# charleschen003/doudizhu-rl

Measured on AMD Instinct MI355X. Metric: env steps/sec (batched tables), higher is better.
Workload: dtype u8; 1 GPU; 65536 tables per GPU, random policy (engine RNG), legal-move list only (no NN), auto-reset: the workload of BASELINE.json configs[1] at the largest single-GPU table count (65,536 per GPU: configs[2] / configs[3]; configs[4] = 8 x 65,536), the same per-GPU workload at every N; tables_per_gpu=65536, total_tables=65536, episodes=2767981, list_layout=slab (fixed-stride segment per table)

## Files before the change

doudizhu-rl_amd/_lib.py:

```python
import ctypes as C
import os

from .build import LIB as _DEFAULT_LIB, LIB_JK as _JK_LIB

_libs = {}

SYMBOLS = {
    "ddz_abi_version": (C.c_int, []),
    "ddz_num_actions": (C.c_int, []),
    "ddz_strerror": (C.c_char_p, [C.c_int]),
    "ddz_last_hip_error": (C.c_int, []),
    "ddz_state_bytes": (C.c_int64, [C.c_int64]),
    "ddz_scratch_bytes": (C.c_int64, [C.c_int64]),
    "ddz_face_planes": (C.c_int, [C.c_int]),
    "ddz_create": (C.c_int, [C.POINTER(C.c_void_p), C.c_int64, C.c_uint64, C.c_uint64, C.c_int,
                             C.c_void_p, C.c_int64, C.c_void_p, C.c_int64]),
    "ddz_destroy": (C.c_int, [C.c_void_p]),
    "ddz_invalidate": (C.c_int, [C.c_void_p]),
    "ddz_reset": (C.c_int, [C.c_void_p, C.c_void_p, C.c_void_p]),
    "ddz_legal": (C.c_int, [C.c_void_p, C.c_void_p, C.c_void_p, C.c_void_p, C.c_int64, C.c_void_p]),
    "ddz_step": (C.c_int, [C.c_void_p, C.c_int, C.c_void_p, C.c_void_p, C.c_void_p, C.c_int,
                           C.c_void_p, C.c_void_p, C.c_void_p, C.c_void_p, C.c_void_p]),
    "ddz_mask_words": (C.c_int, []),
    "ddz_legal_mask": (C.c_int, [C.c_void_p, C.c_void_p, C.c_void_p]),
# ... 54 lines not shown
    "ddz_q_features_needed": (C.c_int, [C.c_int, C.c_void_p, C.c_int64, C.c_int, C.c_void_p, C.c_void_p, C.c_void_p, C.c_void_p,
                                        C.c_void_p, C.c_void_p, C.c_int64, C.c_void_p]),
    "ddz_q_fc1_dense": (C.c_int, [C.c_int, C.c_void_p, C.c_int64, C.c_int64, C.c_void_p, C.c_void_p, C.c_void_p]),
    "ddz_q_fc1_rows": (C.c_int, [C.c_int, C.c_void_p, C.c_void_p, C.c_void_p, C.c_void_p, C.c_void_p, C.c_void_p, C.c_int64,
                                 C.c_void_p]),
    "ddz_q_slab_needed": (C.c_int, [C.c_void_p, C.c_void_p, C.c_void_p, C.c_int64, C.c_void_p, C.c_int64, C.c_void_p,
                                    C.c_void_p, C.c_void_p, C.c_void_p, C.c_int64, C.c_void_p, C.c_void_p]),
    "ddz_q_shared_ws_bytes": (C.c_int64, []),
    "ddz_q_shared_need_ws_bytes": (C.c_int64, [C.c_int64]),
    "ddz_q_shared_need": (C.c_int, [C.c_void_p, C.c_void_p, C.c_void_p, C.c_void_p, C.c_int64, C.c_void_p, C.c_int64, C.c_int64,
                                    C.c_void_p, C.c_void_p, C.c_void_p, C.c_void_p, C.c_void_p]),
    "ddz_q_features_drows": (C.c_int, [C.c_int, C.c_void_p, C.c_int64, C.c_int, C.c_void_p, C.c_void_p, C.c_void_p, C.c_void_p,
                                       C.c_int64, C.c_void_p, C.c_void_p, C.c_void_p, C.c_int64, C.c_void_p]),
    "ddz_q_shared_rows": (C.c_int, [C.c_void_p, C.c_void_p, C.c_int64, C.c_int64, C.c_void_p, C.c_void_p, C.c_void_p, C.c_void_p]),
    "ddz_q_shared_hash_ws_bytes": (C.c_int64, [C.c_int64]),
    "ddz_q_shared_rows_hashed": (C.c_int, [C.c_void_p, C.c_int, C.c_void_p, C.c_int64, C.c_int64, C.c_void_p, C.c_void_p, C.c_void_p,
                                           C.c_void_p]),
    "ddz_q_features_rows": (C.c_int, [C.c_int, C.c_void_p, C.c_int64, C.c_int, C.c_void_p, C.c_void_p, C.c_void_p, C.c_void_p,
                                      C.c_void_p, C.c_int64, C.c_int64, C.c_void_p, C.c_void_p, C.c_void_p]),
    "ddz_q_gather_h0": (C.c_int, [C.c_int, C.c_void_p, C.c_int64, C.c_void_p, C.c_int64, C.c_void_p, C.c_void_p, C.c_void_p]),
    "ddz_q_fc1_rows_k": (C.c_int, [C.c_int, C.c_void_p, C.c_int64, C.c_void_p, C.c_void_p, C.c_void_p, C.c_int64, C.c_int, C.c_void_p]),
    "ddz_q_roles_ws_bytes": (C.c_int64, [C.c_int64, C.c_int, C.c_int]),
    "ddz_q_roles_rows": (C.c_int, [C.c_void_p, C.c_int, C.c_void_p, C.c_int, C.c_void_p, C.c_int64, C.c_int64, C.c_void_p, C.c_void_p,
                                   C.c_void_p, C.c_void_p, C.c_void_p]),
    "ddz_q_roles_features_rows": (C.c_int, [C.c_int, C.c_void_p, C.c_int64, C.c_int, C.c_int, C.c_void_p, C.c_void_p, C.c_void_p,
                                            C.c_void_p, C.c_void_p, C.c_int64, C.c_int64, C.c_void_p]),
    "ddz_q_roles_fc1_rows_k": (C.c_int, [C.c_int, C.c_int, C.c_void_p, C.c_int64, C.c_void_p, C.c_void_p, C.c_void_p, C.c_int64,
                                         C.c_void_p]),
    "ddz_q_roles_gather_h0": (C.c_int, [C.c_int, C.c_int, C.c_void_p, C.c_int64, C.c_void_p, C.c_void_p, C.c_int64, C.c_void_p,
                                        C.c_void_p, C.c_void_p]),
    "ddz_q_roles_need_ws_bytes": (C.c_int64, [C.c_int64, C.c_int]),
    "ddz_q_roles_need": (C.c_int, [C.c_void_p, C.c_int, C.c_void_p, C.c_void_p, C.c_void_p, C.c_int64, C.c_void_p, C.c_int64,
                                   C.c_int64, C.c_void_p, C.c_void_p, C.c_void_p, C.c_void_p, C.c_void_p]),
    "ddz_q_roles_features_drows": (C.c_int, [C.c_int, C.c_void_p, C.c_int64, C.c_int, C.c_int, C.c_void_p, C.c_void_p, C.c_void_p,
                                             C.c_void_p, C.c_int64, C.c_void_p, C.c_void_p, C.c_void_p, C.c_int64, C.c_void_p]),
    "ddz_q_roles_fc1_rows": (C.c_int, [C.c_int, C.c_int, C.c_void_p, C.c_void_p, C.c_void_p, C.c_void_p, C.c_void_p, C.c_void_p,
                                       C.c_int64, C.c_void_p]),
    "ddz_q_roles_slab": (C.c_int, [C.c_void_p, C.c_int, C.c_void_p, C.c_void_p, C.c_void_p, C.c_int64, C.c_void_p, C.c_int64,
                                   C.c_void_p, C.c_void_p, C.c_void_p, C.c_void_p, C.c_int64, C.c_void_p, C.c_void_p]),
    "ddz_action_table": (C.c_int, [C.c_int, C.c_void_p, C.c_void_p]),
    "ddz_pack_trajectory": (C.c_int, [C.c_int, C.c_void_p, C.c_int64, C.c_void_p, C.c_void_p]),
    "ddz_auto_choose_state": (C.c_int, [C.c_void_p, C.c_int, C.c_void_p, C.c_void_p, C.c_void_p]),
    "ddz_auto_choose": (C.c_int, [C.c_int, C.c_void_p, C.c_void_p, C.c_void_p, C.c_int64, C.c_void_p, C.c_void_p,
                                  C.c_void_p]),
    "ddz_debug_cards_value": (C.c_int, [C.c_int, C.c_void_p, C.c_void_p]),
    "ddz_debug_auto_leaf": (C.c_int, [C.c_int, C.c_void_p, C.c_void_p, C.c_int64, C.c_void_p, C.c_void_p, C.c_void_p]),
    "ddz_debug_auto_choose_state": (C.c_int, [C.c_void_p, C.c_int, C.c_int, C.c_void_p, C.c_void_p, C.c_void_p]),
    "ddz_debug_set_geometry": (C.c_int, [C.c_void_p, C.c_int, C.c_int, C.c_int]),
    "ddz_debug_set_auto_teams": (C.c_int, [C.c_void_p, C.c_int]),
    "ddz_status": (C.c_int, [C.c_void_p, C.c_void_p, C.c_void_p]),
    "ddz_sync": (C.c_int, [C.c_int, C.c_void_p]),
    "ddz_device_status": (C.c_int, [C.c_int, C.c_void_p, C.c_void_p]),
    "ddz_debug_classify": (C.c_int, [C.c_int, C.c_void_p, C.c_int64, C.c_void_p, C.c_void_p]),
}


class QSrc(C.Structure):
    _fields_ = [("kind", C.c_int), ("planes", C.c_int), ("face", C.c_void_p), ("action", C.c_void_p), ("variant", C.c_int),
                ("n_actions", C.c_int), ("states", C.c_void_p), ("ids", C.c_void_p), ("index", C.c_void_p), ("table", C.c_void_p),
                ("n_rows", C.c_int64)]


class DdzError(RuntimeError):
    pass


_override = None


def use_library(path):
    global _override
    if False in _libs:
        raise DdzError("use_library() must be called before the library is first used")
    _override = path


def lib(jk=False):
    jk = bool(jk)
    if jk not in _libs:
        LIB = _JK_LIB if jk else (_override or _DEFAULT_LIB)
        if not os.path.exists(LIB):
            raise DdzError(
                f"{LIB} is missing: build it with `python __graft_entry__.py build` "
                "(hipcc --offload-arch=gfx950). There is no CPU fallback.")
        L = C.CDLL(LIB)
        for name, (res, args) in SYMBOLS.items():
            fn = getattr(L, name)
            fn.restype = res
            fn.argtypes = args
        if L.ddz_abi_version() != 1:
            raise DdzError("libddz_hip.so ABI version mismatch")
        if L.ddz_num_actions() != (13551 if jk else 13527):
            raise DdzError(f"{LIB}: unexpected rule set ({L.ddz_num_actions()} actions)")
        _libs[jk] = L
    return _libs[jk]


def check(rc, L=None):
    if rc != 0:
        L = L or lib()
        msg = L.ddz_strerror(rc).decode()
        if rc == -3:
            msg += f" (hipError {L.ddz_last_hip_error()})"
        raise DdzError(f"libddz_hip: {msg}")
```

doudizhu-rl_amd/csrc/ddz_engine.hip:

```cpp
#include <hip/hip_runtime.h>
#include <stddef.h>
#include <stdint.h>
#include <stdlib.h>
#include <string.h>

#include <atomic>
#include <mutex>

#include "../../include/ddz_env.h"
#include "ddz_device.h"

using namespace ddz;

namespace {

constexpr int BLOCK = 256;
constexpr int WPB = 16;
constexpr int TB = WPB * 64;
constexpr int STATE_ROW_BYTES = DDZ_NFIELDS * DDZ_ROW;

constexpr int F_ENUM = 1, F_STEP = 2, F_RESET = 4, F_COUNT = 8, F_SLAB = 16;

constexpr int AUTO_SLOTS = 4;
constexpr int AO_HDR_BYTES = 576;
// ... 414 lines not shown
#pragma unroll
  for (int i = (int)threadIdx.x - OFF; i < HOT_SLOTS; i += NT - OFF) {
    const int id = i < HOT_IDS ? i : ID_BIGBANG;
    hot.meta[i] = g_tab[2 * id + 1];
    if (HT::HAS_ROWS) hot.rows[i] = g_tab[2 * id];
  }
#pragma unroll
  for (int i = (int)threadIdx.x - OFF; i < COMBO_WORDS; i += NT - OFF) {
    if constexpr (HT::HAS_C64) hot.c64[i] = g_c64[i];
    else hot.combo[i] = g_combo[i];
  }
}

__device__ __forceinline__ uint64_t nib_from_cards(uint64_t b) {
  uint64_t x = b & 0x000FFFFFFFFFFFFFull;
  x = x - ((x >> 1) & 0x5555555555555555ull);
  x = (x & 0x3333333333333333ull) + ((x >> 2) & 0x3333333333333333ull);
  return x | (((b >> 52) & 1ull) << 52) | (((b >> 53) & 1ull) << 56);
}
__device__ inline void deal_wave(uint64_t gid, uint32_t episode, uint32_t k0, uint32_t k1, int lane,
                                 uint64_t& o0, uint64_t& o1, uint64_t& o2) {
  const uint4 d = philox4x32_10(make_uint4((uint32_t)gid, (uint32_t)(gid >> 32), episode, (1u << 16) | (uint32_t)(lane >> 2)), k0, k1);
  const int w = lane & 3;
  const uint32_t key = w == 0 ? d.x : w == 1 ? d.y : w == 2 ? d.z : d.w;
  const uint64_t kk = ((uint64_t)key << 6) | (uint32_t)lane;
  int pos = 0;
#pragma unroll 6
  for (int j = 0; j < 54; ++j) pos += rl64(kk, j) < kk ? 1 : 0;
  const bool card = lane < 54;
  o0 = nib_from_cards(__ballot(card && pos < 17));
  o1 = nib_from_cards(__ballot(card && pos >= 17 && pos < 37));
  o2 = nib_from_cards(__ballot(card && pos >= 37));
}

__device__ inline void deal_wave_lds(uint64_t gid, uint32_t episode, uint32_t k0, uint32_t k1, int lane, uint64_t* keys,
                                     uint64_t& o0, uint64_t& o1, uint64_t& o2) {
  const uint4 d = philox4x32_10(make_uint4((uint32_t)gid, (uint32_t)(gid >> 32), episode, (1u << 16) | (uint32_t)(lane >> 2)), k0, k1);
  const int w = lane & 3;
  const uint32_t key = w == 0 ? d.x : w == 1 ? d.y : w == 2 ? d.z : d.w;
  const uint64_t kk = ((uint64_t)key << 6) | (uint32_t)lane;
  keys[lane] = kk;
  __builtin_amdgcn_fence(__ATOMIC_ACQ_REL, "wavefront");
  __builtin_amdgcn_wave_barrier();
  int pos = 0;
#pragma unroll 9
  for (int j = 0; j < 54; j += 2) {
    const ulonglong2 v = *(const ulonglong2*)&keys[j];
    pos += (v.x < kk ? 1 : 0) + (v.y < kk ? 1 : 0);
  }
  const bool card = lane < 54;
  o0 = nib_from_cards(__ballot(card && pos < 17));
  o1 = nib_from_cards(__ballot(card && pos >= 17 && pos < 37));
  o2 = nib_from_cards(__ballot(card && pos >= 37));
}

__device__ __forceinline__ uint32_t last_info(uint64_t n1, int c1, uint64_t n2, int c2) {
  if (n1) return info_of_row(n1, c1);
  if (n2) return info_of_row(n2, c2);
  return mk_info(EMPTY, 0, 1);
}

#ifdef DDZ_STAMP
__device__ unsigned long long* g_stamps = nullptr;
template <int N>
struct Stamps {
  unsigned long long acc[N] = {}, last = __builtin_amdgcn_s_memtime();
  __device__ __forceinline__ void mark(int k) {
    const unsigned long long now = __builtin_amdgcn_s_memtime();
    acc[k] += now - last;
    last = now;
  }
  __device__ __forceinline__ void set(int k, unsigned long long v) { acc[k] = v; }
  __device__ __forceinline__ void store(int64_t slot, bool writer) const {
    if (g_stamps && writer)
      for (int q = 0; q < N; ++q) g_stamps[16 * slot + q] = acc[q];
  }
};
#else
template <int N>
struct Stamps {
  __device__ __forceinline__ void mark(int) {}
  __device__ __forceinline__ void set(int, unsigned long long) {}
  __device__ __forceinline__ void store(int64_t, bool) const {}
};
#endif
#include "ddz_auto.h"
#include "ddz_auto2.h"


struct TableArgs {
  uint8_t* state;
  int64_t T;
  int tpw;
  uint32_t k0, k1;
  uint64_t gid_base;
  int auto_reset;
  const void* sel;
  int32_t* offsets;
  uint4* rows;
  int32_t* ids;
  int64_t cap;
  const int32_t* cur_counts;
  const int32_t* cur_local;
  const int32_t* cur_blk;
  int32_t* nxt_counts;
  int32_t* nxt_local;
// ... 356 lines not shown
      scat = src < 16 ? gsz : (uint32_t)QUADRIC;
    }
    snib = (uint64_t)scat << (4 * sr); svlv = (uint32_t)sr | (1u << 8); ncards = scat;
  }
}
template <bool TRAJ, bool WIDE, class M>
__device__ __forceinline__ void round_pick(M okm, int pre, const uint4& row, int idx, uint32_t gsz, uint4& c, uint64_t& snib,
                                           uint32_t& scat, uint32_t& svlv, uint32_t& ncards) {
  const int src = round_src<WIDE>(okm, pre, idx);
  if (TRAJ) c = make_uint4(rl(row.x, src), rl(row.y, src), rl(row.z, src), rl(row.w, src));
  round_entry<WIDE>(src, gsz, snib, scat, svlv, ncards);
}

struct RolloutArgs {
  uint8_t* state;
  int64_t T;
  int tpw;
  uint32_t k0, k1;
  uint64_t gid_base;
  int32_t* counts;
  uint4* rows;
  int32_t* ids;
  int64_t stride;
  int64_t it_rows;
  int64_t it_counts;
  int64_t n_iters;
  uint4* traj;
  int64_t* wave_stats;
  int32_t* status;
  int64_t* legal_rows;
};

template <bool IDS, bool TRAJ, bool STAGED = false, int RW = WPB>
__global__ __launch_bounds__(RW * 64, RW == WPB ? 4 : 6) void k_rollout(RolloutArgs a) {
  Stamps<12> stamps;
  __shared__ HotTabT<false> hot;
  __shared__ uint64_t s_stage[RW][STAGE_CAP];
  __shared__ uint16_t s_svl[RW][STAGE_CAP];
  __shared__ uint16_t s_sid[IDS ? RW : 1][IDS ? STAGE_CAP : 1];
  const int lane = threadIdx.x & 63;
  const int wv = (int)rfl(threadIdx.x >> 6);
  const int64_t wave = (int64_t)blockIdx.x * RW + wv;
  const int64_t t0 = wave * a.tpw;
  const int ntab = t0 < a.T ? (int)(a.T - t0 < a.tpw ? a.T - t0 : a.tpw) : 0;
  uint4 Rnext = make_uint4(0, 0, 0, 0);
  if (ntab > 0 && lane < DDZ_NFIELDS) Rnext = ((const uint4*)(a.state + t0 * STATE_ROW_BYTES))[lane];
  hot_fill<RW * 64>(hot);
  __syncthreads();
  uint64_t* stage = s_stage[wv];
  uint16_t* svl = s_svl[wv];
  uint16_t* sid = s_sid[IDS ? wv : 0];
  int s_ply = 0;
  int64_t s_rows = 0;
  const FastLanes fl = fast_lanes(lane);
  for (int i = 0; i < ntab; ++i) {
    const int64_t t = t0 + i;
    stamps.mark(0);
    uint4* trow = (uint4*)(a.state + t * STATE_ROW_BYTES);
    const uint4 R = Rnext;
    if (i + 1 < ntab && lane < DDZ_NFIELDS) Rnext = ((const uint4*)(a.state + (t + 1) * STATE_ROW_BYTES))[lane];
    const uint64_t gid = a.gid_base + (uint64_t)t;
    uint64_t P = pack_row(R);
    uint32_t aux = R.w >> 24;
    const uint32_t mx = rl(R.x, DDZ_F_META), my = rl(R.y, DDZ_F_META), mz = rl(R.z, DDZ_F_META);
    const uint32_t my_hi = my & 0xFFFF0000u;
    uint32_t mw = rl(R.w, DDZ_F_META);
    int role = mx & 0xFF;
    if (role > 2) role = 0;
    const bool active = ((my >> 16) & 0xFF) && !((mx >> 8) & 0xFF);
    uint32_t ply = my & 0xFFFF, episode = mz;
    uint64_t hc = rl64(P, DDZ_F_HAND0 + role), hn = rl64(P, DDZ_F_HAND0 + (role == 2 ? 0 : role + 1)),
             hp = rl64(P, DDZ_F_HAND0 + (role == 0 ? 2 : role - 1));
    uint32_t trick = mk_info(EMPTY, 0, 1);
    int passes = 0;
    {
      const int rm1 = role == 0 ? 2 : role - 1, rp1 = role == 2 ? 0 : role + 1;
      const uint64_t n1 = rl64(P, DDZ_F_RECENT0 + rm1), n2 = rl64(P, DDZ_F_RECENT0 + rp1);
      if (n1) trick = info_of_row(n1, (int)rl(aux, DDZ_F_RECENT0 + rm1));
      else if (n2) { trick = info_of_row(n2, (int)rl(aux, DDZ_F_RECENT0 + rp1)); passes = 1; }
    }
    uint32_t draws = 0, dnext = 64;
    uint4* tj = TRAJ ? a.traj + 2 * t : nullptr;
    if (!active) {
      if (lane == 0) {
        a.counts[t] = 0;
        if (STAGED)
          for (int64_t j = 1; j < a.n_iters; ++j) a.counts[t + j * a.it_counts] = 0;
      }
      if (TRAJ) {
        const uint4 f0 = make_uint4(0, 0, 0, 0);
        const uint4 f1 = make_uint4((uint32_t)role | ((mx >> 8) & 0xFF) << 8 | 2u << 24, ply << 16, episode, 0xFFFFFFFFu);
        for (int it = (int)a.n_iters; it > 0; --it) {
          if (lane < 2) tj[lane] = sel4(lane == 0, f0, f1);
          tj += 2 * a.T;
        }
      }
      continue;
    }
    int idle = 0;
    for (int it = (int)a.n_iters; it > 0; --it) {
      uint4 tr0 = make_uint4(0, 0, 0, 0);
      uint4 tr1 = make_uint4((uint32_t)role, ply << 16, episode, 0xFFFFFFFFu);
      uint32_t dn = rfl(dnext);
      if (dn >= 64u) {
        dn = 0;
        dnext = 0;
// ... 90 lines not shown
          *cnt_p = n;
          s_rows += n;
          const int64_t tbase = base + n0;
          for (int j = lane; j < n - n0; j += 64) {
            const uint64_t e = stage[j];
            a.rows[tbase + j] = unpack_row(e & 0x0FFFFFFFFFFFFFFFull, (uint32_t)(e >> 60));
            if (IDS) a.ids[tbase + j] = sid[j];
          }
          stamps.mark(3);
          if (n > 0) {
            idx = (int)rfl(__umulhi(draw, (uint32_t)n));
            if (idx < n0) {
              if (lead) round_entry<true>(round_src<true>(okm, round_pre(okm), idx), 0u, snib, scat, svlv, ncards);
              else round_entry<false>(round_src<false>((uint32_t)okm, round_pre((uint32_t)okm), idx), (uint32_t)lc0, snib, scat, svlv, ncards);
              if (TRAJ) c = unpack_row(snib, scat);
            } else {
              const uint64_t e = stage[idx - n0];
              const uint64_t anib = e & 0x0FFFFFFFFFFFFFFFull;
              const uint32_t acat = (uint32_t)(e >> 60);
              if (TRAJ) c = unpack_row(anib, acat);
              snib = (uint64_t)rfl((uint32_t)anib) | ((uint64_t)rfl((uint32_t)(anib >> 32)) << 32);
              scat = rfl(acat);
              svlv = rfl((uint32_t)svl[idx - n0]);
              ncards = (uint32_t)nib_sum(snib);
            }
          }
          stamps.mark(10);
        }
      }
      tr1.y |= (uint32_t)n & 0xFFFF;
      if (n <= 0) {
        tr1.x |= 2u << 24;
        idle += 1;
      } else {
        {
          const int d = lane - role;
          const uint64_t add = (d == DDZ_F_HIST0 || lane == DDZ_F_TAKEN) ? snib : 0ull;
          P = d == DDZ_F_RECENT0 ? snib : P + add;
          aux = d == DDZ_F_RECENT0 ? scat : d == DDZ_F_HAND0 ? aux - ncards : aux;
        }
        stamps.mark(6);
        const uint64_t hnew = hand - snib;
        if (snib) { trick = scat | (svlv << 8); passes = 0; } else { passes += 1; }
        constexpr bool WON_SCALAR = !(STAGED && RW != WPB && DDZ_NATIVE_JOKER_KICKERS);
        const bool won = WON_SCALAR ? rfl((uint32_t)hnew | (uint32_t)(hnew >> 32)) == 0u : hnew == 0;
        const uint32_t o_reward = won ? (role == 1 ? 0xFFu : 1u) : 0u;
        tr0 = c;
        tr1.x |= (uint32_t)won << 8 | o_reward << 16;
        tr1.w = (uint32_t)idx;
        ply += 1;
        dnext += 1;
        stamps.mark(7);
        if (won) {
          if (lane == 0) {
            int64_t* ws = a.wave_stats + 4 * wave;
            ws[1] += 1;
            ws[2] += role == 1 ? 1ll : role == 0 ? (1ll << 32) : 0ll;
          }
          episode += 1;
          uint32_t dk0 = a.k0, dk1 = a.k1;
          asm volatile("" : "+s"(dk0), "+s"(dk1));
          uint64_t h0, h1, h2;
#ifdef DDZ_ROLLOUT_DEAL_READLANE
          deal_wave(gid, episode, dk0, dk1, lane, h0, h1, h2);
#else
          deal_wave_lds(gid, episode, dk0, dk1, lane, stage, h0, h1, h2);
#endif
          hc = h1; hn = h2; hp = h0;
          P = 0;
          aux = lane == 1 ? 20u : lane < 3 ? 17u : 0u;
          mw = 0;
          role = 1; ply = 0; trick = mk_info(EMPTY, 0, 1); passes = 0; dnext = 64;
        } else {
          role = role == 2 ? 0 : role + 1;
          hc = hn; hn = hp; hp = hnew;
        }
        stamps.mark(8);
      }
      if (TRAJ && lane < 2) tj[lane] = sel4(lane == 0, tr0, tr1);
      if (TRAJ) tj += 2 * a.T;
      stamps.mark(4);
      __builtin_amdgcn_wave_barrier();
    }
    s_ply += (int)a.n_iters - idle;
    if (idle < (int)a.n_iters) {
      const int rp1 = role == 2 ? 0 : role + 1, rm1 = role == 0 ? 2 : role - 1;
      const uint64_t Pf = lane == role ? hc : lane == rp1 ? hn : lane == rm1 ? hp : P;
      uint4 Rf = unpack_row(Pf, aux);
      if (lane == DDZ_F_META) Rf = make_uint4((uint32_t)role | (0xFFu << 16), ply == 0 ? 1u << 16 : my_hi | (ply & 0xFFFF), episode, mw);
      if (lane < DDZ_NFIELDS) trow[lane] = Rf;
    }
    stamps.mark(9);
  }
  stamps.store(t0, lane == 0 && ntab > 0);
  if (ntab > 0 && lane == 0) {
    int64_t* ws = a.wave_stats + 4 * wave;
    ws[0] += s_ply; ws[3] += s_rows;
  }
}

#include "ddz_playout.h"

__device__ __forceinline__ void store_stream(float4* p, const float4 v) {
  __builtin_nontemporal_store(v.x, &p->x);
  __builtin_nontemporal_store(v.y, &p->y);
  __builtin_nontemporal_store(v.z, &p->z);
  __builtin_nontemporal_store(v.w, &p->w);
}

struct SlabArgs {
  uint8_t* state;
  int64_t T;
  int tpw;
  uint32_t k0, k1;
  uint64_t gid_base;
  int auto_reset;
  const void* sel;
  int32_t* counts;
  uint4* rows;
  int32_t* ids;
  int64_t stride;
  uint8_t* done;
  int8_t* reward;
  uint8_t* illegal;
  uint4* traj;
  int64_t* wave_stats;
  int32_t* status;
  uint64_t thr;
  int32_t* choice_out;
  float4* face;
  int face_variant;
  int coop;
  int team;
  int lpt;
};
constexpr int STEP_Q = 4;

template <bool IDS, class HT>
__device__ __forceinline__ int slab_list(uint64_t hand, uint32_t info, int64_t base, int64_t stride, uint4* rows, int32_t* ids,
                                         const HT& hot, int lane, const FastLanes& fl, int32_t* status) {
  const int lc0 = (int)(info & 0xFF);
  int n;
  if (hand != 0 && lc0 != EMPTY && lc0 <= TRIPLE && !(info & (QF_FROZEN | QF_BADLAST))) {
    const int lv0 = (int)((info >> 8) & 0xFF);
    const int cntr = lane < 15 ? (int)((hand >> (4 * (lane & 15))) & 15) : 0;
    const uint32_t mlc = (uint32_t)__ballot(cntr >= lc0) & (lc0 == SINGLE ? M15 : M13);
    const uint32_t mq = (uint32_t)__ballot(cntr >= 4) & M13;
    const bool rocket = ((uint32_t)__ballot(cntr >= 1) & JOKERS) == JOKERS;
    const uint32_t okm = 1u | ((mlc & gt_mask(lv0)) << 1) | (mq << 16) | (rocket ? 1u << 29 : 0u);
    n = __builtin_popcount(okm);
// ... 366 lines not shown
        wr &= wr - 1;
        const uint32_t ep = rl(episode, i) + 1u;
        uint64_t h0, h1, h2;
        deal_wave(a.gid_base + (uint64_t)(t0 + i), ep, a.k0, a.k1, lane, h0, h1, h2);
        if (lane < DDZ_NFIELDS)
          srow[i * DDZ_NFIELDS + lane] = lane == 0 ? unpack_row(h0, 17) : lane == 1 ? unpack_row(h1, 20) : lane == 2 ? unpack_row(h2, 17)
                                         : lane == DDZ_F_META ? make_uint4(1u | (0xFFu << 16), 1u << 16, ep, 0) : make_uint4(0, 0, 0, 0);
        if (lane == i) { qhand = h1; qinfo = LEAD; }
      }
      __builtin_amdgcn_fence(__ATOMIC_ACQ_REL, "wavefront");
      __builtin_amdgcn_wave_barrier();
      const uint64_t stm = chm & ~deferred;
      if (lane < nrows && ((stm >> (lane / DDZ_NFIELDS)) & 1)) sp[lane] = srow[lane];
      if (64 + lane < nrows && ((stm >> ((64 + lane) / DDZ_NFIELDS)) & 1)) sp[64 + lane] = srow[64 + lane];
      if (128 + lane < nrows && ((stm >> ((128 + lane) / DDZ_NFIELDS)) & 1)) sp[128 + lane] = srow[128 + lane];
    }
    if (coop && valid)
      s_share[lane] = deal_l ? make_uint4(deal_ep, 0u, LEAD, 3u)
                             : make_uint4((uint32_t)qhand, (uint32_t)(qhand >> 32), qinfo, live ? 1u : 0u);
    }
    stamps.mark(3);
    if (first || lpt) __syncthreads();
    if (lpt) {
      if (live) {
        const int lc = (int)(qinfo & 0xFF);
        const bool lead = lc == EMPTY;
        const bool rich = __builtin_popcount(ge_mask(qhand, 3)) >= 2 || ge_mask(qhand, 4) != 0;
        const int cls = deal_l ? 0 : lead ? (rich ? 0 : 1) : lc <= TRIPLE ? 3 : 2;
        const int pos = atomicAdd(&s_wcnt[cls], 1);
        s_work[cls][pos] = deal_l ? make_uint4(deal_ep, 0u, LEAD, (uint32_t)(t - tblk0) | 0x80000000u)
                                  : make_uint4((uint32_t)qhand, (uint32_t)(qhand >> 32), qinfo, (uint32_t)(t - tblk0));
      }
      __syncthreads();
    }
    if (MODE == STEP_Q && a.face && face_first && ntab > 0) {
      face_phase(srow, ntab, lane, a.face, a.face_variant, t0);
      stamps.mark(6);
    }
    int n_l = 0;
    if (coop) {
      stamps.mark(1);
      bool heavy = false;
      if (wv < cn) {
        const uint4 sh = s_share[wv];
        const uint32_t fw = rfl(sh.w);
        const int64_t tt = tb0 + wv;
        int n = 0;
        if (fw & 1u) {
          uint64_t hand = (uint64_t)rfl(sh.x) | ((uint64_t)rfl(sh.y) << 32);
          const uint32_t qi = rfl(sh.z);
          if (fw & 2u) {
            const uint32_t ep = rfl(sh.x);
            uint64_t h0, h1, h2;
            deal_wave_lds(a.gid_base + (uint64_t)tt, ep, a.k0, a.k1, lane, s_keys[wv], h0, h1, h2);
            if (lane < DDZ_NFIELDS)
              ((uint4*)(a.state + tt * STATE_ROW_BYTES))[lane] =
                  lane == 0 ? unpack_row(h0, 17) : lane == 1 ? unpack_row(h1, 20) : lane == 2 ? unpack_row(h2, 17)
                  : lane == DDZ_F_META ? make_uint4(1u | (0xFFu << 16), 1u << 16, ep, 0) : make_uint4(0, 0, 0, 0);
            hand = h1;
            stamps.mark(7);
          }
          const int thr = a.team;
          if (thr && hand != 0 && (qi & 0xFF) == EMPTY && !(qi & (QF_FROZEN | QF_BADLAST)) &&
              (__builtin_popcount(ge_mask(hand, 3)) >= 2 || ge_mask(hand, 4) != 0)) {
            const Out o{a.rows, a.ids, tt * a.stride, (tt + 1) * a.stride, nullptr, nullptr, nullptr};
            stamps.mark(4);
            Pick pk{-1, 0, 0, 0, 0};
            pk.desc = s_desc[wv];
            plan_scan_t<EM_TEAM_PLAN, IDS, true>(hand, follow_of(qi), hot, lane, o, pk);
            __builtin_amdgcn_fence(__ATOMIC_ACQ_REL, "wavefront");
            __builtin_amdgcn_wave_barrier();
            const int R = pk.rc;
            stamps.mark(8);
            if (R > TEAM_ROUNDS) {
              if (lane == 0 && a.status) atomicOr(a.status, 2);
            } else if (R >= thr) {
              heavy = true;
              if (lane == 0) s_item[atomicAdd(&s_nheavy, 1)] = make_uint4((uint32_t)hand, (uint32_t)(hand >> 32), (uint32_t)R, (uint32_t)wv);
            } else {
              const uint64_t hand8 = hand | 0x8888888888888888ull;
              for (int r = 0; r < R; ++r)
                n += team_round<true, IDS>(s_desc[wv][r], hand8, hot, lane, o.base + n, o.cap, a.rows, a.ids);
              if (n > a.stride) {
                if (lane == 0 && a.status) atomicOr(a.status, 2);
                n = 0;
              }
              stamps.mark(9);
            }
          } else {
            n = slab_list<IDS>(hand, qi, tt * a.stride, a.stride, a.rows, a.ids, hot, lane, fl, a.status);
          }
        }
        if (lane == 0 && !heavy) a.counts[tt] = n;
        s_rows += n;
      }
      stamps.mark(4);
      __syncthreads();
      const int nh = s_nheavy;
      stamps.mark(6);
      if (nh > 0) {
        for (int h = 0; h < nh; ++h) {
          const uint4 e = s_item[h];
          const uint64_t hand8 = ((uint64_t)rfl(e.x) | ((uint64_t)rfl(e.y) << 32)) | 0x8888888888888888ull;
          const int R = (int)rfl(e.z), ow = (int)rfl(e.w);
          for (int r = (wv + 5 * h) & (WPB - 1); r < R; r += WPB) {
            const int k = team_round<false, IDS>(s_desc[ow][r], hand8, hot, lane, 0, 0, a.rows, a.ids);
            if (lane == 0) s_tcnt[ow][r] = (uint32_t)k;
// ... 2 lines not shown
        stamps.mark(10);
        __syncthreads();
        if (wv < nh) {
          const uint4 e = s_item[wv];
          const int R = (int)rfl(e.z), ow = (int)rfl(e.w);
          int run = 0;
          for (int r0 = 0; r0 < R; r0 += 64) {
            const int i = r0 + lane;
            const int v = i < R ? (int)s_tcnt[ow][i] : 0;
            const int inc = wave_scan_add(v);
            if (i < R) s_tcnt[ow][i] = (uint32_t)v | (uint32_t)(run + inc - v) << 16;
            run += (int)rl((uint32_t)inc, 63);
          }
          if (run > a.stride) {
            if (lane == 0 && a.status) atomicOr(a.status, 2);
            run = 0;
          }
          if (lane == 0) a.counts[tb0 + ow] = run;
          s_rows += run;
        }
        __syncthreads();
        for (int h = 0; h < nh; ++h) {
          const uint4 e = s_item[h];
          const uint64_t hand8 = ((uint64_t)rfl(e.x) | ((uint64_t)rfl(e.y) << 32)) | 0x8888888888888888ull;
          const int R = (int)rfl(e.z), ow = (int)rfl(e.w);
          const int64_t base = (tb0 + ow) * a.stride;
          for (int r = (wv + 5 * h) & (WPB - 1); r < R; r += WPB) {
            const uint32_t cb = rfl(s_tcnt[ow][r]);
            if (cb & 0xFFFFu)
              team_round<true, IDS>(s_desc[ow][r], hand8, hot, lane, base + (int)(cb >> 16), base + a.stride, a.rows, a.ids);
          }
        }
      }
      stamps.mark(11);
    }
    if (lpt) {
      const int n0 = s_wcnt[0], n1 = n0 + s_wcnt[1], n2 = n1 + s_wcnt[2], n3 = n2 + s_wcnt[3];
      for (;;) {
        int k = 0;
        if (lane == 0) k = atomicAdd(&s_wcnt[WL_CLASSES], 1);
        k = (int)rfl((uint32_t)k);
        if (k >= n3) break;
        const int cls = k < n0 ? 0 : k < n1 ? 1 : k < n2 ? 2 : 3;
        const uint4 e = s_work[cls][k - (cls == 0 ? 0 : cls == 1 ? n0 : cls == 2 ? n1 : n2)];
        const uint32_t ew = rfl(e.w);
        const int64_t tt = tblk0 + (int64_t)(ew & 0x7FFFFFFFu);
        uint64_t hand = (uint64_t)rfl(e.x) | ((uint64_t)rfl(e.y) << 32);
        if (ew >> 31) {
          const uint32_t ep = rfl(e.x);
          uint64_t h0, h1, h2;
#ifdef DDZ_SLAB_DEAL_READLANE
          deal_wave(a.gid_base + (uint64_t)tt, ep, a.k0, a.k1, lane, h0, h1, h2);
#else
          deal_wave_lds(a.gid_base + (uint64_t)tt, ep, a.k0, a.k1, lane, (uint64_t*)srow, h0, h1, h2);
#endif
          if (lane < DDZ_NFIELDS)
            ((uint4*)(a.state + tt * STATE_ROW_BYTES))[lane] =
                lane == 0 ? unpack_row(h0, 17) : lane == 1 ? unpack_row(h1, 20) : lane == 2 ? unpack_row(h2, 17)
                : lane == DDZ_F_META ? make_uint4(1u | (0xFFu << 16), 1u << 16, ep, 0) : make_uint4(0, 0, 0, 0);
          hand = h1;
        }
        const int n = slab_list<IDS>(hand, rfl(e.z), tt * a.stride, a.stride, a.rows, a.ids, hot, lane, fl, a.status);
        if (lane == 0) a.counts[tt] = n;
        s_rows += n;
      }
    }
    uint64_t lv = (coop || lpt) ? 0ull : __ballot(live);
    while (lv) {
      const int i = __builtin_ctzll(lv);
      lv &= lv - 1;
      const int n = slab_list<IDS>(rl64(qhand, i), rl(qinfo, i), (t0 + i) * a.stride, a.stride, a.rows, a.ids, hot, lane, fl,
                                   a.status);
      if (lane == i) n_l = n;
      s_rows += n;
    }
    if (MODE == STEP_Q && a.face && !face_first && ntab > 0) {
      face_phase(srow, ntab, lane, a.face, a.face_variant, t0);
      __builtin_amdgcn_fence(__ATOMIC_ACQ_REL, "wavefront");
      __builtin_amdgcn_wave_barrier();
      stamps.mark(6);
    }
    if (valid) {
      if (lpt) { if (!live) a.counts[t] = 0; }
      else if (!coop) a.counts[t] = n_l;
      if (a.done) a.done[t] = (uint8_t)o_done;
      if (a.reward) a.reward[t] = (int8_t)o_reward;
      if (a.illegal) a.illegal[t] = (uint8_t)o_illegal;
    }
    stamps.mark(4);
    first = false;
  }
  stamps.set(5, (unsigned long long)(coop ? 1 : nw));
  stamps.store(coop ? tb0 + wv : tw0, lane == 0 && (coop ? wv < cn : nw > 0));
  if ((coop ? wv < cn : (nw > 0 || lpt)) && lane == 0) {
    int64_t* ws = a.wave_stats + 4 * wave;
    ws[0] += s_ply; ws[1] += s_eps; ws[2] += (int64_t)s_lord | ((int64_t)s_up << 32); ws[3] += s_rows;
  }
}

template <bool IDS>
__global__ __launch_bounds__(TB, 4) void k_moves_slab(const uint4* __restrict__ hands, const uint4* __restrict__ lasts,
                                                      int64_t n, int tpw, int32_t* __restrict__ counts,
                                                      uint4* __restrict__ rows, int32_t* __restrict__ ids, int64_t stride,
                                                      int32_t* __restrict__ status) {
  __shared__ HotTabL hot;
  const int lane = threadIdx.x & 63;
  const int wv = (int)rfl(threadIdx.x >> 6);
// ... 267 lines not shown
template <int P>
__global__ __launch_bounds__(QH) void k_q_feat(const float4* __restrict__ face, int64_t T, const float* __restrict__ wf,
                                               const float* __restrict__ bias, const float* __restrict__ acnt,
                                               float* __restrict__ y, int64_t ystride) {
  const int c = threadIdx.x;
  __shared__ float4 s_face[QF_TILE * P * 15];
  const int64_t tb = (int64_t)blockIdx.x * QF_TILE;
  const int nt = (int)(T - tb < QF_TILE ? T - tb : QF_TILE);
  for (int i = threadIdx.x; i < nt * P * 15; i += QH) s_face[i] = face[tb * P * 15 + i];
  float w[P][10];
#pragma unroll
  for (int p = 0; p < P; ++p) {
    int q = 0;
#pragma unroll
    for (int k = 0; k < 4; ++k)
#pragma unroll
      for (int j = 0; j <= k; ++j) w[p][q++] = wf[(int64_t)(p * 4 + j) * (4 * QH) + k * QH + c];
  }
  float b[4], a[4][4];
#pragma unroll
  for (int k = 0; k < 4; ++k) {
    b[k] = bias[k * QH + c];
#pragma unroll
    for (int n = 0; n < 4; ++n) a[n][k] = acnt[((n + 1) * 4 + k) * QH + c];
  }
  __syncthreads();
  const int64_t cs = T * ystride;
  for (int r = 0; r < 15; ++r) {
    const int ncnt = r < 13 ? 4 : 1;
    float* dst = y + ((int64_t)r * 5 * T + tb) * ystride + c;
    for (int ti = 0; ti < nt; ++ti) {
      float s0 = b[0], s1 = b[1], s2 = b[2], s3 = b[3];
#pragma unroll
      for (int p = 0; p < P; ++p) {
        const float4 x = s_face[(ti * P + p) * 15 + r];
        q_feat_plane(w[p], x, s0, s1, s2, s3);
      }
      float* d = dst + ti * ystride;
      d[0] = fmaxf(fmaxf(s0, s1), fmaxf(s2, s3));
      for (int n = 0; n < ncnt; ++n)
        d[(n + 1) * cs] = fmaxf(fmaxf(s0 + a[n][0], s1 + a[n][1]), fmaxf(s2 + a[n][2], s3 + a[n][3]));
    }
  }
}

#include "ddz_qnet.h"

__global__ __launch_bounds__(BLOCK) void k_classify(const uint4* __restrict__ rows, int64_t n,
                                                    uint32_t* __restrict__ out) {
  const int64_t t = (int64_t)blockIdx.x * BLOCK + threadIdx.x;
  if (t < n) out[t] = classify(pack_row(rows[t]));
}

__global__ __launch_bounds__(BLOCK) void k_reduce_stats(Scratch sc, int64_t nslots, int64_t* stats) {
  __shared__ long long sh[5][BLOCK];
  long long v[5] = {0, 0, 0, 0, 0};
  for (int64_t b = threadIdx.x; b < nslots; b += BLOCK) {
    const long long w = sc.blk_stats[4 * b + 2];
    v[0] += sc.blk_stats[4 * b]; v[1] += sc.blk_stats[4 * b + 1]; v[3] += sc.blk_stats[4 * b + 3];
    v[2] += w & 0xFFFFFFFFll; v[4] += w >> 32;
    for (int k = 0; k < 4; ++k) sc.blk_stats[4 * b + k] = 0;
  }
  for (int k = 0; k < 5; ++k) sh[k][threadIdx.x] = v[k];
  __syncthreads();
  for (int d = BLOCK / 2; d > 0; d >>= 1) {
    if ((int)threadIdx.x < d)
      for (int k = 0; k < 5; ++k) sh[k][threadIdx.x] += sh[k][threadIdx.x + d];
    __syncthreads();
  }
  if (threadIdx.x == 0) {
    stats[0] += sh[0][0];
    stats[1] += sh[1][0];
    stats[2] += *sc.legal_rows + sh[3][0];
    stats[3] += sh[2][0];
    stats[4] += sh[4][0];
    stats[5] += sh[1][0] - sh[2][0] - sh[4][0];
    *sc.legal_rows = 0;
  }
}


template <int P>
__device__ __forceinline__ void face_split(int64_t idx, int64_t n, int64_t& t, int& rem) {
  if (n * (P * 15) <= 0x7FFFFFFFll) {
    const uint32_t i32 = (uint32_t)idx, t32 = i32 / (uint32_t)(P * 15);
    t = t32;
    rem = (int)(i32 - t32 * (uint32_t)(P * 15));
  } else {
    t = idx / (P * 15);
    rem = (int)(idx - t * (P * 15));
  }
}

template <int VARIANT>
__device__ __forceinline__ float4 face_cell(const uint8_t* __restrict__ row, int rem) {
  constexpr uint64_t KINDS = VARIANT == 0 ? 0x8710ull : VARIANT == 1 ? 0x8743210ull
                           : VARIANT == 2 ? 0x876543210ull : 0x876510ull;
  const int p = rem / 15, i = rem - p * 15;
  auto byte = [&](int f, int k) { return (int)row[f * 16 + k]; };
  int role = byte(DDZ_F_META, 0);
  if (role > 2) role = 0;
  const int kind = (int)((KINDS >> (4 * p)) & 15);
  const int rm1 = role == 0 ? 2 : role - 1, rp1 = role == 2 ? 0 : role + 1;
  float4 v;
  if (kind < 7) {
    const int f = kind == 0 ? DDZ_F_HAND0 + role : kind == 1 ? DDZ_F_TAKEN
// ... 1688 lines not shown
int ddz_q_roles_slab(ddz_env_t* e, int n_nets, const int8_t* slot, const float* h0, const float* d, int64_t d_rows, const int32_t* row_index,
                     int64_t hidden, const float* w2, const float* b2, const int32_t* counts, const int8_t* rows, int64_t stride, float* q,
                     void* stream) {
  if (!good(e)) return DDZ_EHANDLE;
  if (!al(h0, 16) || !al(d, 16) || !al(w2, 16) || !al(b2, 4) || !al(counts, 4) || !al(rows, 16) || !al(q, 4) || !al(row_index, 4))
    return DDZ_EINVAL;
  if (!roles_ok(n_nets) || !slot || !h0 || !d || !w2 || !b2 || !counts || !rows || !q || !row_index || hidden != QH || stride < 1 || d_rows < 1)
    return DDZ_EINVAL;
  DeviceGuard g(e->device);
  if (!g.ok) return DDZ_ENODEV;
  int tpw;
  const dim3 grid = q_slab_grid(e->T, tpw);
  hipLaunchKernelGGL(k_q_slab_roles, grid, dim3(TB), 0, (hipStream_t)stream,
                     (const float4*)h0, (const float4*)d, d_rows, e->T, tpw, (const float4*)w2, b2, slot, counts, (const uint4*)rows,
                     stride, q, row_index, e->sc.status);
  return check_launch();
}

int ddz_action_table(int device, int8_t* rows, void* stream) {
  if (!al(rows, 16)) return DDZ_EINVAL;
  if (!rows) return DDZ_EINVAL;
  DeviceGuard g(device);
  if (!g.ok) return DDZ_ENODEV;
  int rc = ensure_table(device);
  if (rc) return rc;
  hipLaunchKernelGGL(k_export_table, dim3((NUM_ACTIONS_X + BLOCK - 1) / BLOCK), dim3(BLOCK), 0, (hipStream_t)stream,
                     (uint4*)rows);
  return check_launch();
}

int ddz_pack_trajectory(int device, const uint8_t* traj, int64_t n_records, uint8_t* packed, void* stream) {
  if (!al(traj, 16) || !al(packed, 8)) return DDZ_EINVAL;
  if (n_records < 0 || (n_records > 0 && (!traj || !packed))) return DDZ_EINVAL;
  if (n_records == 0) return DDZ_OK;
  DeviceGuard g(device);
  if (!g.ok) return DDZ_ENODEV;
  int rc = ensure_table(device);
  if (rc) return rc;
  hipLaunchKernelGGL(k_pack_traj, dim3((unsigned)((n_records + BLOCK - 1) / BLOCK)), dim3(BLOCK), 0, (hipStream_t)stream,
                     (const uint4*)traj, n_records, (uint2*)packed);
  return check_launch();
}

int ddz_debug_classify(int device, const int8_t* rows, int64_t n, uint32_t* out, void* stream) {
  if (!al(rows, 16) || !al(out, 4)) return DDZ_EINVAL;
  if (n <= 0 || !rows || !out) return DDZ_EINVAL;
  DeviceGuard g(device);
  if (!g.ok) return DDZ_ENODEV;
  hipLaunchKernelGGL(k_classify, dim3((unsigned)((n + BLOCK - 1) / BLOCK)), dim3(BLOCK), 0, (hipStream_t)stream,
                     (const uint4*)rows, n, out);
  return check_launch();
}

}
```

include/ddz_env.h:

```cpp
#ifndef DDZ_ENV_H
#define DDZ_ENV_H
#include <stdint.h>

#ifdef __cplusplus
extern "C" {
#endif

#define DDZ_ABI_VERSION 1
#define DDZ_NUM_ACTIONS 13527
#define DDZ_ROW 16
#define DDZ_NFIELDS 11
#define DDZ_TRAJ_BYTES 32
#define DDZ_SLAB_MIN_STRIDE 512

#define DDZ_OK 0
#define DDZ_EINVAL (-1)
#define DDZ_EHANDLE (-2)
#define DDZ_EHIP (-3)
#define DDZ_ECAP (-4)
#define DDZ_ENODEV (-5)

enum { DDZ_F_HAND0 = 0, DDZ_F_HIST0 = 3, DDZ_F_RECENT0 = 6, DDZ_F_TAKEN = 9, DDZ_F_META = 10 };

#define DDZ_STEP_RANDOM 0
// ... 158 lines not shown
int ddz_q_shared_rows_hashed(ddz_env_t* env, int variant, void* ws, int64_t ws_bytes, int64_t row_capacity, int32_t* rows,
                             int32_t* rep, int32_t* seg, void* stream);
int ddz_q_features_rows(int device_id, const float* face, int64_t n_tables, int planes, const float* wf, const float* bias,
                        const int32_t* rep, const int32_t* seg, float* ys, int64_t ys_ld, int64_t row_capacity, const float* mz,
                        float* g, void* stream);
int ddz_q_gather_h0(int device_id, const float* g, int64_t g_rows, const int32_t* rows, int64_t n_tables, const float* base,
                    float* h0, void* stream);
int ddz_q_fc1_rows_k(int device_id, const float* y, int64_t k, const int32_t* seg, const float* w2k, float* g,
                     int64_t row_capacity, int accumulate, void* stream);

int64_t ddz_q_roles_ws_bytes(int64_t n_tables, int variant, int n_nets);
int ddz_q_roles_rows(ddz_env_t* env, int variant, const int32_t* net_of_role, int n_nets, void* ws, int64_t ws_bytes,
                     int64_t row_capacity, int32_t* rows, int32_t* rep, int32_t* seg, int8_t* slot, void* stream);
int ddz_q_roles_features_rows(int device_id, const float* face, int64_t n_tables, int planes, int n_nets, const float* wf,
                              const float* bias, const int32_t* rep, const int32_t* seg, float* ys, int64_t ys_ld,
                              int64_t row_capacity, void* stream);
int ddz_q_roles_fc1_rows_k(int device_id, int n_nets, const float* y, int64_t k, const int32_t* seg, const float* w2k, float* g,
                           int64_t row_capacity, void* stream);
int ddz_q_roles_gather_h0(int device_id, int n_nets, const float* g, int64_t g_rows, const int32_t* rows, const int8_t* slot,
                          int64_t n_tables, const float* base, float* h0, void* stream);
int64_t ddz_q_roles_need_ws_bytes(int64_t shared_row_capacity, int n_nets);
int ddz_q_roles_need(ddz_env_t* env, int n_nets, const int32_t* row_index, const int32_t* rows, const int32_t* sseg,
                     int64_t shared_row_capacity, void* ws, int64_t ws_bytes, int64_t row_capacity, int32_t* row_index2,
                     int32_t* drep, int32_t* dseg, uint8_t* row_cnt, void* stream);
int ddz_q_roles_features_drows(int device_id, const float* face, int64_t n_tables, int planes, int n_nets, const float* wf,
                               const float* bias, const float* acnt, const int32_t* rep, int64_t shared_row_capacity,
                               const int32_t* drep, const int32_t* dseg, float* dy, int64_t row_capacity, void* stream);
int ddz_q_roles_fc1_rows(int device_id, int n_nets, const float* dy, const int32_t* seg, const uint8_t* row_cnt, const float* w2,
                         const float* z, float* d, int64_t row_capacity, void* stream);
int ddz_q_roles_slab(ddz_env_t* env, int n_nets, const int8_t* slot, const float* h0, const float* d, int64_t d_rows,
                     const int32_t* row_index, int64_t hidden, const float* w2, const float* b2, const int32_t* counts,
                     const int8_t* rows, int64_t stride, float* q, void* stream);

int ddz_action_table(int device_id, int8_t* rows, void* stream);

#define DDZ_TRAJ_PACKED_BYTES 8
int ddz_pack_trajectory(int device_id, const uint8_t* traj, int64_t n_records, uint8_t* packed, void* stream);

int ddz_auto_choose_state(ddz_env_t* env, int auto_roles, int32_t* ids, int64_t* stats, void* stream);
int ddz_auto_choose(int device_id, const int8_t* hands, const int8_t* lasts, const uint8_t* info, int64_t n,
                    int32_t* ids, int64_t* stats, void* stream);
int ddz_debug_cards_value(int device_id, int8_t* out, void* stream);
int ddz_debug_auto_leaf(int device_id, const int32_t* in, const double* rp, int64_t n, double* value, int32_t* move, void* stream);
int ddz_debug_auto_choose_state(ddz_env_t* env, int kernel, int auto_roles, int32_t* ids, int64_t* stats, void* stream);
int ddz_debug_set_geometry(ddz_env_t* env, int tables_per_wave, int slab_coop, int slab_work_list);
int ddz_debug_set_auto_teams(ddz_env_t* env, int on);

int ddz_status(ddz_env_t* env, int32_t* status_out, void* stream);
int ddz_device_status(int device_id, int32_t* status_out, void* stream);
int ddz_sync(int device_id, void* stream);

int ddz_debug_classify(int device_id, const int8_t* rows, int64_t n, uint32_t* out, void* stream);

#ifdef __cplusplus
}
#endif
#endif
```

Before: 4.894 billion env steps/s.

## Rank deal keys as 32-bit values with exact tie fallback; register episode stats

```diff
diff --git a/doudizhu-rl_amd/_lib.py b/doudizhu-rl_amd/_lib.py
--- a/doudizhu-rl_amd/_lib.py
+++ b/doudizhu-rl_amd/_lib.py
@@ -130,6 +130,7 @@
     "ddz_sync": (C.c_int, [C.c_int, C.c_void_p]),
     "ddz_device_status": (C.c_int, [C.c_int, C.c_void_p, C.c_void_p]),
     "ddz_debug_classify": (C.c_int, [C.c_int, C.c_void_p, C.c_int64, C.c_void_p, C.c_void_p]),
+    "ddz_debug_deal_rank": (C.c_int, [C.c_int, C.c_void_p, C.c_int64, C.c_void_p, C.c_void_p, C.c_void_p]),
 }
 
 
diff --git a/doudizhu-rl_amd/csrc/ddz_engine.hip b/doudizhu-rl_amd/csrc/ddz_engine.hip
--- a/doudizhu-rl_amd/csrc/ddz_engine.hip
+++ b/doudizhu-rl_amd/csrc/ddz_engine.hip
@@ -490,6 +490,49 @@
   o0 = nib_from_cards(__ballot(card && pos < 17));
   o1 = nib_from_cards(__ballot(card && pos >= 17 && pos < 37));
   o2 = nib_from_cards(__ballot(card && pos >= 37));
+}
+
+__device__ inline bool deal_rank_lds32(const uint32_t* kw, int lane, uint64_t& o0, uint64_t& o1, uint64_t& o2) {
+  const uint32_t key = kw[lane];
+  const bool card = lane < 54;
+  int pos = 0;
+  constexpr int G = 2;
+#pragma unroll
+  for (int g = 0; g < 14; g += G) {
+    uint4 v[G];
+    asm volatile("" ::: "memory");
+#pragma unroll
+    for (int q = 0; q < G; ++q)
+      if (g + q < 14) v[q] = ((const uint4*)kw)[g + q];
+#pragma unroll
+    for (int q = 0; q < G; ++q)
+      if (g + q < 14) pos += (v[q].x < key ? 1 : 0) + (v[q].y < key ? 1 : 0) + (v[q].z < key ? 1 : 0) + (v[q].w < key ? 1 : 0);
+  }
+  uint64_t b0 = __ballot(card && pos < 17), b1 = __ballot(card && pos >= 17 && pos < 37);
+  const bool exact = !(__builtin_popcountll(b0) == 17 && __builtin_popcountll(b1) == 20);
+  if (exact) {
+    const uint64_t kk = ((uint64_t)key << 6) | (uint32_t)lane;
+    pos = 0;
+#pragma unroll 1
+    for (int j = 0; j < 54; ++j) pos += (((uint64_t)kw[j] << 6) | (uint32_t)j) < kk ? 1 : 0;
+    b0 = __ballot(card && pos < 17);
+    b1 = __ballot(card && pos >= 17 && pos < 37);
+  }
+  o0 = nib_from_cards(b0);
+  o1 = nib_from_cards(b1);
+  o2 = nib_from_cards(~(b0 | b1) & ((1ull << 54) - 1));
+  return exact;
+}
+
+__device__ inline void deal_wave_lds32(uint64_t gid, uint32_t episode, uint32_t k0, uint32_t k1, int lane, uint32_t* kw,
+                                       uint64_t& o0, uint64_t& o1, uint64_t& o2) {
+  const uint4 d = philox4x32_10(make_uint4((uint32_t)gid, (uint32_t)(gid >> 32), episode, (1u << 16) | (uint32_t)(lane >> 2)), k0, k1);
+  const int w = lane & 3;
+  const uint32_t key = w == 0 ? d.x : w == 1 ? d.y : w == 2 ? d.z : d.w;
+  kw[lane] = lane < 54 ? key : 0xFFFFFFFFu;
+  __builtin_amdgcn_fence(__ATOMIC_ACQ_REL, "wavefront");
+  __builtin_amdgcn_wave_barrier();
+  deal_rank_lds32(kw, lane, o0, o1, o2);
 }
 
 __device__ __forceinline__ uint32_t last_info(uint64_t n1, int c1, uint64_t n2, int c2) {
@@ -952,6 +995,8 @@
   uint16_t* sid = s_sid[IDS ? wv : 0];
   int s_ply = 0;
   int64_t s_rows = 0;
+  constexpr bool STATS_REG = RW == WPB || (!TRAJ && !STAGED);
+  int s_eps = 0, s_lord = 0, s_up = 0;
   const FastLanes fl = fast_lanes(lane);
   for (int i = 0; i < ntab; ++i) {
     const int64_t t = t0 + i;
@@ -1148,7 +1193,11 @@
         dnext += 1;
         stamps.mark(7);
         if (won) {
-          if (lane == 0) {
+          if (STATS_REG) {
+            s_eps += 1;
+            s_lord += role == 1 ? 1 : 0;
+            s_up += role == 0 ? 1 : 0;
+          } else if (lane == 0) {
             int64_t* ws = a.wave_stats + 4 * wave;
             ws[1] += 1;
             ws[2] += role == 1 ? 1ll : role == 0 ? (1ll << 32) : 0ll;
@@ -1159,14 +1208,24 @@
           uint64_t h0, h1, h2;
 #ifdef DDZ_ROLLOUT_DEAL_READLANE
           deal_wave(gid, episode, dk0, dk1, lane, h0, h1, h2);
+          dnext = 64;
 #else
-          deal_wave_lds(gid, episode, dk0, dk1, lane, stage, h0, h1, h2);
+          const bool kl = lane < 14;
+          uint4 d = philox4x32_10(make_uint4((uint32_t)gid, (uint32_t)(gid >> 32), episode,
+                                             kl ? (1u << 16) | (uint32_t)lane : (2u << 16) | (uint32_t)(lane - 14)), dk0, dk1);
+          draws = d.x;
+          if (lane == 13) d.z = d.w = 0xFFFFFFFFu;
+          if (kl) ((uint4*)stage)[lane] = d;
+          __builtin_amdgcn_fence(__ATOMIC_ACQ_REL, "wavefront");
+          __builtin_amdgcn_wave_barrier();
+          deal_rank_lds32((const uint32_t*)stage, lane, h0, h1, h2);
+          dnext = 14;
 #endif
           hc = h1; hn = h2; hp = h0;
           P = 0;
           aux = lane == 1 ? 20u : lane < 3 ? 17u : 0u;
           mw = 0;
-          role = 1; ply = 0; trick = mk_info(EMPTY, 0, 1); passes = 0; dnext = 64;
+          role = 1; ply = 0; trick = mk_info(EMPTY, 0, 1); passes = 0;
         } else {
           role = role == 2 ? 0 : role + 1;
           hc = hn; hn = hp; hp = hnew;
@@ -1192,6 +1251,7 @@
   if (ntab > 0 && lane == 0) {
     int64_t* ws = a.wave_stats + 4 * wave;
     ws[0] += s_ply; ws[3] += s_rows;
+    if (STATS_REG) { ws[1] += s_eps; ws[2] += (int64_t)s_lord | ((int64_t)s_up << 32); }
   }
 }
 
@@ -1664,7 +1724,7 @@
           if (fw & 2u) {
             const uint32_t ep = rfl(sh.x);
             uint64_t h0, h1, h2;
-            deal_wave_lds(a.gid_base + (uint64_t)tt, ep, a.k0, a.k1, lane, s_keys[wv], h0, h1, h2);
+            deal_wave_lds32(a.gid_base + (uint64_t)tt, ep, a.k0, a.k1, lane, (uint32_t*)s_keys[wv], h0, h1, h2);
             if (lane < DDZ_NFIELDS)
               ((uint4*)(a.state + tt * STATE_ROW_BYTES))[lane] =
                   lane == 0 ? unpack_row(h0, 17) : lane == 1 ? unpack_row(h1, 20) : lane == 2 ? unpack_row(h2, 17)
@@ -1773,7 +1833,7 @@
 #ifdef DDZ_SLAB_DEAL_READLANE
           deal_wave(a.gid_base + (uint64_t)tt, ep, a.k0, a.k1, lane, h0, h1, h2);
 #else
-          deal_wave_lds(a.gid_base + (uint64_t)tt, ep, a.k0, a.k1, lane, (uint64_t*)srow, h0, h1, h2);
+          deal_wave_lds32(a.gid_base + (uint64_t)tt, ep, a.k0, a.k1, lane, (uint32_t*)srow, h0, h1, h2);
 #endif
           if (lane < DDZ_NFIELDS)
             ((uint4*)(a.state + tt * STATE_ROW_BYTES))[lane] =
@@ -2147,6 +2207,23 @@
   if (t < n) out[t] = classify(pack_row(rows[t]));
 }
 
+__global__ __launch_bounds__(BLOCK) void k_deal_rank(const uint32_t* __restrict__ keys, int64_t n, uint64_t* __restrict__ hands,
+                                                     int32_t* __restrict__ path) {
+  __shared__ uint4 s_kw[BLOCK / 64][16];
+  const int lane = threadIdx.x & 63;
+  const int wv = (int)rfl(threadIdx.x >> 6);
+  const int64_t s = (int64_t)blockIdx.x * (BLOCK / 64) + wv;
+  if (s >= n) return;
+  uint32_t* kw = (uint32_t*)s_kw[wv];
+  kw[lane] = lane < 54 ? keys[s * 54 + lane] : 0xFFFFFFFFu;
+  __builtin_amdgcn_fence(__ATOMIC_ACQ_REL, "wavefront");
+  __builtin_amdgcn_wave_barrier();
+  uint64_t h0, h1, h2;
+  const bool exact = deal_rank_lds32(kw, lane, h0, h1, h2);
+  if (lane < 3) hands[3 * s + lane] = lane == 0 ? h0 : lane == 1 ? h1 : h2;
+  if (lane == 0) path[s] = exact ? 1 : 0;
+}
+
 __global__ __launch_bounds__(BLOCK) void k_reduce_stats(Scratch sc, int64_t nslots, int64_t* stats) {
   __shared__ long long sh[5][BLOCK];
   long long v[5] = {0, 0, 0, 0, 0};
@@ -3941,4 +4018,15 @@
   return check_launch();
 }
 
-}
+
+int ddz_debug_deal_rank(int device, const uint32_t* keys, int64_t n, uint64_t* hands, int32_t* path, void* stream) {
+  if (!al(keys, 4) || !al(hands, 8) || !al(path, 4)) return DDZ_EINVAL;
+  if (n <= 0 || !keys || !hands || !path) return DDZ_EINVAL;
+  DeviceGuard g(device);
+  if (!g.ok) return DDZ_ENODEV;
+  constexpr int SETS = BLOCK / 64;
+  hipLaunchKernelGGL(k_deal_rank, dim3((unsigned)((n + SETS - 1) / SETS)), dim3(BLOCK), 0, (hipStream_t)stream, keys, n, hands, path);
+  return check_launch();
+}
+
+}
diff --git a/include/ddz_env.h b/include/ddz_env.h
--- a/include/ddz_env.h
+++ b/include/ddz_env.h
@@ -234,6 +234,8 @@
 
 int ddz_debug_classify(int device_id, const int8_t* rows, int64_t n, uint32_t* out, void* stream);
 
+int ddz_debug_deal_rank(int device_id, const uint32_t* keys, int64_t n, uint64_t* hands, int32_t* path, void* stream);
+
 #ifdef __cplusplus
 }
 #endif
```

Result: no change. 4.929 billion env steps/s, median of 6 (+0.7%).
